# arangesh/Ground-Plane-Polling

Hardware: AMD Instinct MI355X
Metric: images/sec end-to-end (resnet50, 1k planes, 1242x375) (higher is better)
Workload: dtype f16x3

## Files before the change

### ground-plane-polling_amd/csrc/conv_igemm.hip

```cpp

#include <hip/hip_runtime.h>
#include <stdint.h>
#include <stdlib.h>

#include "conv_igemm_types.h"
#include "gpp.h"

namespace {

inline bool is_x3(int dtype) { return dtype == GPP_BF16X3 || dtype == GPP_F16X3; }
inline bool f32_storage(int dtype) { return dtype == GPP_F32 || is_x3(dtype); }
inline int elem_size(int dtype) { return f32_storage(dtype) ? 4 : 2; }

int validate(const gpp_conv_desc& d)
{
    if (!d.in || !d.weight || !d.out) return GPP_ERR_BAD_ARG;
    if (d.dtype != GPP_BF16 && d.dtype != GPP_F16 && d.dtype != GPP_F32 && !is_x3(d.dtype)) return GPP_ERR_UNSUPPORTED;
    const int esz = elem_size(d.dtype), ck = 128 / esz, va = 16 / esz;
    if (d.batch <= 0 || d.C_in <= 0 || d.C_out <= 0 || d.KH <= 0 || d.KW <= 0) return GPP_ERR_BAD_ARG;
    constexpr int kMaxDim = 1 << 20;
    if (d.batch > kMaxDim || d.C_in > kMaxDim || d.C_out > kMaxDim || d.in_pitch > kMaxDim || d.out_pitch > kMaxDim || d.res_pitch > kMaxDim ||
        d.weight_rows > kMaxDim || d.weight_rows < 0 || d.in_pitch < 0 || d.out_pitch < 0 || d.res_pitch < 0 || d.partial_bytes < 0)
        return GPP_ERR_UNSUPPORTED;
    if (d.KH > 8 || d.KW > 8) return GPP_ERR_UNSUPPORTED;
// ... 138 lines not shown
{
    return block_entry(conv1x1_a, conv3x3_b, conv1x1_c, tile, stream);
}

extern "C" int gpp_bottleneck_tail(const gpp_conv_desc* conv3x3, const gpp_conv_desc* conv1x1, int tile_rows, void* stream)
{
    return tail_entry(conv3x3, conv1x1, tile_rows, stream);
}

extern "C" int gpp_x3_range_events(uint64_t* host_count, int reset)
{
    unsigned long long v = 0;
    const int rc = gpp_x3_range_events_f16x3(&v, reset);
    if (rc == GPP_OK && host_count) *host_count = (uint64_t)v;
    return rc;
}

extern "C" int gpp_x3_range_snapshot(uint64_t* device_count, void* stream)
{
    return gpp_x3_range_snapshot_of(nullptr, device_count, stream);
}

extern "C" int gpp_x3_range_snapshot_of(const uint64_t* counter, uint64_t* device_count, void* stream)
{
    if (!device_count) return GPP_ERR_BAD_ARG;
    if (((uintptr_t)counter | (uintptr_t)device_count) & 7) return GPP_ERR_ALIGN;
    return gpp_x3_range_snapshot_f16x3((const unsigned long long*)counter, (unsigned long long*)device_count, (hipStream_t)stream);
}

extern "C" int gpp_conv2d_flops(const gpp_conv_desc* host_desc, double* flops)
{
    if (!host_desc || !flops) return GPP_ERR_BAD_ARG;
    if (host_desc->n_groups < 1 || host_desc->n_groups > GPP_MAX_GROUPS) return GPP_ERR_BAD_ARG;
    double f = 0.0;
    for (int g = 0; g < host_desc->n_groups; ++g)
        f += 2.0 * host_desc->batch * (double)host_desc->groups[g].H_out * host_desc->groups[g].W_out *
             host_desc->KH * host_desc->KW * (double)host_desc->C_in * host_desc->C_out;
    *flops = f;
    return GPP_OK;
}

extern "C" int gpp_conv2d_split_rule(const gpp_conv_desc* host_desc, int* split_k)
{
    if (!host_desc || !split_k) return GPP_ERR_BAD_ARG;
    gpp_conv_desc d = *host_desc;
    int rc = validate(d);
    if (rc != GPP_OK) return rc;
    *split_k = d.split_k > 0 ? d.split_k : split_rule(d);
    return GPP_OK;
}

extern "C" int gpp_conv2d_workspace_bytes(const gpp_conv_desc* host_desc, size_t* bytes)
{
    if (!host_desc || !bytes) return GPP_ERR_BAD_ARG;
    gpp_conv_desc d = *host_desc;
    char probe[16] __attribute__((aligned(16)));
    if (!d.partial) { d.partial = probe; d.partial_bytes = 0; }
    int rc = validate(d);
    if (rc != GPP_OK) return rc;
    const int split = d.split_k > 0 ? d.split_k : split_rule(d);
    *bytes = 0;
    if (split <= 1) return GPP_OK;
    int64_t rows = 0;
    for (int g = 0; g < d.n_groups; ++g) rows += (int64_t)d.batch * d.groups[g].H_out * d.groups[g].W_out + 256;
    const int64_t npad = (d.C_out + 255) / 256 * 256;
    *bytes = (size_t)(split * rows * npad * 4);
    return GPP_OK;
}

extern "C" int gpp_conv2d_igemm(const gpp_conv_desc* host_desc, void* stream)
{
    if (!host_desc) return GPP_ERR_BAD_ARG;
    gpp_conv_desc d = *host_desc;
    for (int g = 0; g < GPP_MAX_GROUPS; ++g) d.groups[g].row_begin = 0;
    int rc = validate(d);
    if (rc != GPP_OK) return rc;
    return dispatch_any(d, (hipStream_t)stream);
}

static const int kTiles[] = {0, 64064, 96064, 128064, 160064, 192064, 64128, 96128, 128128, 160128, 192128, 224128,
                             1128128, 1192128, 1128256, 1160256, 1192256, 1224256, 256256, 1256256,
                             128160, 192160, 1192160, 1128160, 2256256, 1192096, 3256224, 3192160, 4128064, 4064064, 4128128, 4064128,
                             5064064, 5096064, 5064128, 5096128, 5128128,
                             128256, 192256};
static bool tile_is_candidate(const gpp_conv_desc* desc, int tile)
{
    const int ck = 128 / elem_size(desc->dtype);
    const int nk = desc->KH * desc->KW * (desc->C_in / ck);
    int64_t rows = 0;
    for (int g = 0; g < desc->n_groups; ++g) rows += (int64_t)desc->batch * desc->groups[g].H_out * desc->groups[g].W_out;
    const int bn = tile % 1000 ? tile % 1000 : 128;
    if (tile >= 5000000) {
        static const bool no_deep = [] { const char* e = getenv("GPP_NO_DEEP_TILES"); return e && e[0] == '1'; }();
        const bool x3_in = is_x3(desc->dtype) && (desc->x3_split & GPP_X3_IN);
        const int bm = (tile / 1000) % 1000;
        int64_t tiles_m = 0;
        for (int g = 0; g < desc->n_groups; ++g) tiles_m += ((int64_t)desc->batch * desc->groups[g].H_out * desc->groups[g].W_out + bm - 1) / bm;
        const int64_t wgs = tiles_m * ((desc->C_out + bn - 1) / bn) * (desc->split_k > 1 ? desc->split_k : 1);
        if (bn == 64 && desc->C_out > 256) return false;
        return !no_deep && x3_in && nk >= 12 && wgs <= 320;
    }
    if (tile >= 4000000) {
        static const bool no_ws = [] { const char* e = getenv("GPP_NO_WS_TILES"); return e && e[0] == '1'; }();
        const bool x3_in = is_x3(desc->dtype) && (desc->x3_split & GPP_X3_IN);
        const int bm = (tile / 1000) % 1000;
        const gpp_conv_group& G = desc->groups[0];
        return !no_ws && x3_in && desc->KH == 1 && desc->KW == 1 && desc->stride == 1 && desc->pad_top == 0 && desc->pad_left == 0 && desc->n_groups == 1 &&
               desc->split_k <= 1 && desc->C_out % bn == 0 && 32 % (desc->C_out / bn) == 0 && G.H_in == G.H_out && G.W_in == G.W_out &&
               (!desc->residual || ((desc->x3_split & GPP_X3_RES) && G.H_res == G.H_out && G.W_res == G.W_out)) &&
               (desc->C_in / 32) * bn * 128 + 4 * bm * 128 <= 160 * 1024 && rows >= 256 * 16;
    }
    static const bool no_mix = [] { const char* e = getenv("GPP_NO_MIX_TILES"); return e && e[0] == '1'; }();
    if (tile >= 3000000 && no_mix) return false;
    if (tile >= 3000000) {
        const bool x3_in = is_x3(desc->dtype) && (desc->x3_split & GPP_X3_IN);
        return x3_in && desc->C_out % 256 == 0 && nk >= 4 && desc->split_k <= 1 && rows * (desc->C_out / 256) >= 256 * 256;
    }
    if (tile && bn == 64 && desc->C_out > 256 && !(desc->KH == 1 && desc->KW == 1 && desc->C_in <= 256)) return false;
    if (bn == 256 && (desc->C_out < 192 || rows < 256 * 16)) return false;
    const bool x3_pipe = is_x3(desc->dtype) && (desc->x3_split & GPP_X3_IN);
    if (tile > 1000000 && tile < 3000000 && (nk < 4 || (f32_storage(desc->dtype) && !x3_pipe))) return false;
    if ((tile == 1256256 || tile == 1160256 || tile == 1224256) && !x3_pipe) return false;
    if (x3_pipe && tile == 1192160) return false;
    if (bn == 256 && desc->dtype == GPP_F32) return false;
    if ((tile == 128256 || tile == 192256) && !is_x3(desc->dtype)) return false;
    if (bn == 160 && (desc->C_out + 159) / 160 * 160 >= (desc->C_out + 127) / 128 * 128) return false;
    if (bn == 96 && (desc->C_out + 95) / 96 * 96 >= (desc->C_out + 127) / 128 * 128) return false;
    if (tile == 2256256 && (desc->C_out < 384 || desc->C_out % 256 != 128 || rows < 256 * 16)) return false;
    return true;
}

extern "C" int gpp_conv2d_tile_candidates(const gpp_conv_desc* desc, int* tiles, int capacity, int* count)
{
    if (!desc || !count || capacity < 0 || (capacity > 0 && !tiles)) return GPP_ERR_BAD_ARG;
    {
        gpp_conv_desc d = *desc;
        for (int g = 0; g < GPP_MAX_GROUPS; ++g) d.groups[g].row_begin = 0;
        const int rc = validate(d);
        if (rc != GPP_OK) return rc;
    }
    int n = 0;
    for (int tile : kTiles) {
        if (!tile_is_candidate(desc, tile)) continue;
        if (n < capacity) tiles[n] = tile;
        ++n;
    }
    *count = n;
    return GPP_OK;
}

extern "C" int gpp_conv2d_autotune(gpp_conv_desc* desc, int iters, void* stream, float* best_us)
{
    if (!desc || iters < 1) return GPP_ERR_BAD_ARG;
    {
        gpp_conv_desc d = *desc;
        for (int g = 0; g < GPP_MAX_GROUPS; ++g) d.groups[g].row_begin = 0;
        const int rc = validate(d);
        if (rc != GPP_OK) return rc;
    }
    hipStream_t st = (hipStream_t)stream;
    hipEvent_t e0, e1;
    hipError_t e = hipEventCreate(&e0);
    if (e != hipSuccess) return (int)e;
    e = hipEventCreate(&e1);
    if (e != hipSuccess) { (void)hipEventDestroy(e0); return (int)e; }
    const int tile_in = desc->tile_hint;
    float best = 1e30f;
    int best_tile = tile_in, rc = GPP_OK;
    auto time_one = [&](int tile, float* us, int reps = 2) -> int {
        desc->tile_hint = tile;
        int r = gpp_conv2d_igemm(desc, stream);
        if (r != GPP_OK) return r;
        float t_best = 1e30f;
        for (int rep = 0; rep < reps; ++rep) {
// ... 41 lines not shown
```

### ground-plane-polling_amd/csrc/conv_igemm_impl.h

```cpp
#ifndef GPP_CONV_IGEMM_IMPL_H_
#define GPP_CONV_IGEMM_IMPL_H_

#include <hip/hip_runtime.h>
#include <stdint.h>

#include <atomic>

#include "gpp.h"

namespace {

typedef __attribute__((ext_vector_type(8))) __bf16 bf16x8;
typedef __attribute__((ext_vector_type(8))) _Float16 f16x8;
typedef __attribute__((ext_vector_type(4))) float f32x4;

struct f32x8 {
    f32x4 lo, hi;
    __device__ __forceinline__ float operator[](int e) const { return e < 4 ? lo[e] : hi[e - 4]; }
};

template <int DT> struct Elem;
template <> struct Elem<GPP_BF16> {
    using scalar = __bf16;
    using vec8 = bf16x8;
// ... 1769 lines not shown
    };
    rows_of(0, obase, rbase, valid);
    fetch_res(rbase);

    f32x4 acc[MF][NF];
    for (int c = 0; c < my_tiles; ++c) {
#pragma unroll
        for (int i = 0; i < MF; ++i)
#pragma unroll
            for (int j = 0; j < NF; ++j) acc[i][j] = (f32x4){0.f, 0.f, 0.f, 0.f};
        int slot = (c * nk) & (R - 1);
        for (int ks = 0; ks < nk; ++ks) {
            if (ks == 0) asm volatile("s_waitcnt vmcnt(0)" ::: "memory");
            else asm volatile("s_waitcnt vmcnt(%0)" ::"n"((D - 1) * A_IT) : "memory");
            asm volatile("s_waitcnt lgkmcnt(0)" ::: "memory");
            __builtin_amdgcn_s_barrier();
            asm volatile("" ::: "memory");
            issue();
            const unsigned char* sa = ring + slot * SLAB;
            const unsigned char* sw = wbase + ks * BN * kRowBytes;
            xh8 ah[MF], al[MF], bh[NF], bl[NF];
#pragma unroll
            for (int i = 0; i < MF; ++i) {
                ah[i] = *(const xh8*)(sa + a_rd[0] + i * 16 * kRowBytes);
                al[i] = *(const xh8*)(sa + a_rd[1] + i * 16 * kRowBytes);
            }
#pragma unroll
            for (int j = 0; j < NF; ++j) {
                bh[j] = *(const xh8*)(sw + b_rd[0] + j * 16 * kRowBytes);
                bl[j] = *(const xh8*)(sw + b_rd[1] + j * 16 * kRowBytes);
            }
#pragma unroll
            for (int i = 0; i < MF; ++i)
#pragma unroll
                for (int j = 0; j < NF; ++j) {
                    const int js = GPP_SERP2(i, j, NF);
                    acc[i][js] = X3Half<DT>::mfma(bl[js], ah[i], acc[i][js]);
                    acc[i][js] = X3Half<DT>::mfma(bh[js], ah[i], acc[i][js]);
                }
#pragma unroll
            for (int i = 0; i < MF; ++i)
#pragma unroll
                for (int j = 0; j < NF; ++j) { const int js = GPP_SERP2(i, j, NF); acc[i][js] = X3Half<DT>::mfma(bh[js], al[i], acc[i][js]); }
            slot = (slot + 1) & (R - 1);
        }
        float v[MF][NG][8];
#pragma unroll
        for (int i = 0; i < MF; ++i)
#pragma unroll
            for (int jj = 0; jj < NG; ++jj) {
#pragma unroll
                for (int e = 0; e < 4; ++e) {
                    if constexpr (OSCALE) {
                        v[i][jj][e] = __builtin_fmaf(acc[i][2 * jj][e], scale_v[jj][e], bias_v[jj][e]);
                        v[i][jj][4 + e] = __builtin_fmaf(acc[i][2 * jj + 1][e], scale_v[jj][4 + e], bias_v[jj][4 + e]);
                    } else {
                        v[i][jj][e] = acc[i][2 * jj][e] + bias_v[jj][e];
                        v[i][jj][4 + e] = acc[i][2 * jj + 1][e] + bias_v[jj][4 + e];
                    }
                }
                if constexpr (HASRES) {
                    float r[8];
                    x3_unpack<DT>(rpre[i][jj].lo, rpre[i][jj].hi, r);
#pragma unroll
                    for (int e = 0; e < 8; ++e) v[i][jj][e] += r[e];
                }
            }
        int64_t ob_next[MF], rb_next[MF];
        bool ok_next[MF];
        if (c + 1 < my_tiles) {
            rows_of(c + 1, ob_next, rb_next, ok_next);
            fetch_res(rb_next);
        }
#pragma unroll
        for (int i = 0; i < MF; ++i)
            if (valid[i]) {
#pragma unroll
                for (int jj = 0; jj < NG; ++jj) finish8_pre<DT>(d, v[i][jj], n + 32 * jj, obase[i], false, f32x8());
            }
        if (c + 1 < my_tiles) {
#pragma unroll
            for (int i = 0; i < MF; ++i) { obase[i] = ob_next[i]; rbase[i] = rb_next[i]; valid[i] = ok_next[i]; }
        }
    }
}

struct DeviceOnce {
    std::atomic<uint64_t> mask{0};
    template <typename K>
    int configure(K kernel, int lds)
    {
        int dev = 0;
        hipError_t e = hipGetDevice(&dev);
        if (e != hipSuccess) return (int)e;
        const uint64_t bit = 1ull << (dev & 63);
        if (mask.load(std::memory_order_acquire) & bit) return GPP_OK;
        e = hipFuncSetAttribute((const void*)kernel, hipFuncAttributeMaxDynamicSharedMemorySize, lds);
        if (e != hipSuccess) return (int)e;
        mask.fetch_or(bit, std::memory_order_release);
        return GPP_OK;
    }
};

template <int DT, int BM, int BN, int WM, int WN, int STAGES, bool PIPE, bool XIN = false>
int launch(gpp_conv_desc& d, hipStream_t st)
{
    if constexpr (kX3<DT> && !XIN) {
        if (d.x3_split & GPP_X3_IN) return launch<DT, BM, BN, WM, WN, STAGES, PIPE, true>(d, st);
    }
    constexpr int BMS = stage_rows(BM, WM * WN);
    constexpr int lds = STAGES * (BMS + BN) * kRowBytes;
    constexpr int CK = kRowBytes / Elem<DT>::ESZ;
    static DeviceOnce once;
    auto kernel = conv_igemm_kernel<DT, BM, BN, WM, WN, STAGES, PIPE, XIN>;
    int rc = once.configure(kernel, lds);
    if (rc != GPP_OK) return rc;
    const int tiles = prepare<BM, BN>(d);
    if (tiles < 0) return tiles;
    const int n_tiles = (d.C_out + BN - 1) / BN;
    const int nk = d.KH * d.KW * (d.C_in / CK);
    int nsplit = 1;
    if (d.split_k > 1) {
        nsplit = d.split_k;
        if (nk / nsplit < 1) return GPP_ERR_BAD_ARG;
        const int64_t slab = (int64_t)tiles * BM * n_tiles * BN * 4;
        if (!d.partial || slab * nsplit > (int64_t)d.partial_bytes) return GPP_ERR_WORKSPACE;
    }
    const int steps = (nk + nsplit - 1) / nsplit;
    const int lds_used = PIPE ? lds : (steps < STAGES ? steps : STAGES) * (BMS + BN) * kRowBytes;
    kernel<<<dim3((unsigned)(tiles * n_tiles), (unsigned)nsplit), dim3(64 * WM * WN), lds_used, st>>>(d);
    if (nsplit > 1) {
        const int64_t total = (int64_t)d.partial_rows * ((d.C_out + 7) / 8);
        splitk_reduce_kernel<DT><<<dim3((unsigned)((total + 255) / 256)), dim3(256), 0, st>>>(d, BM, n_tiles * BN, nsplit);
    }
    hipError_t e = hipGetLastError();
    return e == hipSuccess ? GPP_OK : (int)e;
}

template <int DT>
int launch_dual(const gpp_conv_desc& d, hipStream_t st)
{
    constexpr bool X3 = kX3<DT>;
    constexpr int ESZ = Elem<DT>::ESZ, CK = kRowBytes / ESZ;
    if (X3 && !(d.x3_split & GPP_X3_IN)) return GPP_ERR_UNSUPPORTED;
    if (d.C_out < 384 || d.C_out % 256 != 128 || d.KH * d.KW * (d.C_in / CK) < 2 || d.split_k > 1) return GPP_ERR_UNSUPPORTED;
    constexpr int lds = 2 * (512 + 128) * kRowBytes;
    static DeviceOnce once;
    auto kernel = conv_igemm_dual_kernel<DT, X3>;
    int rc = once.configure(kernel, lds);
    if (rc != GPP_OK) return rc;
    const int head = d.C_out - 128;
    gpp_conv_desc d0 = d, d1 = d;
    d0.C_out = head;
    d1.C_out = 128;
    d1.weight = (const char*)d.weight + (int64_t)head * d.KH * d.KW * d.C_in * ESZ;
    d1.weight_rows = d.weight_rows - head;
    if (d.bias) d1.bias = d.bias + head;
    if (d.out_scale) d1.out_scale = d.out_scale + head;
    for (int g = 0; g < d.n_groups; ++g) {
        d1.groups[g].out_off += head;
        d1.groups[g].res_off += head;
    }
    const int t0 = prepare<256, 256>(d0), t1 = prepare<512, 128>(d1);
    if (t0 < 0) return t0;
    if (t1 < 0) return t1;
    const int n0 = t0 * (head / 256), n1 = t1;
// ... 4 lines not shown
}

template <int DT, int BMA, int BMB>
int launch_mix(const gpp_conv_desc& d, hipStream_t st)
{
    constexpr int BN = 256, CUS = 256;
    constexpr int ESZ = Elem<DT>::ESZ, CK = kRowBytes / ESZ;
    static_assert(kX3<DT>, "mixed grids exist for the x3 types");
    if (!(d.x3_split & GPP_X3_IN)) return GPP_ERR_UNSUPPORTED;
    if (d.C_out % BN != 0 || d.KH * d.KW * (d.C_in / CK) < 2 || d.split_k > 1) return GPP_ERR_UNSUPPORTED;
    const int n_tiles = d.C_out / BN;
    const int64_t rows0 = (int64_t)d.batch * d.groups[0].H_out * d.groups[0].W_out;
    auto tiles_b = [&](int64_t begin, int bm) {
        int64_t t = (rows0 - begin + bm - 1) / bm;
        for (int g = 1; g < d.n_groups; ++g) t += ((int64_t)d.batch * d.groups[g].H_out * d.groups[g].W_out + bm - 1) / bm;
        return t * n_tiles;
    };
    int64_t best_cost = (tiles_b(0, BMA) + CUS - 1) / CUS * BMA;
    int best_ra = 0;
    for (int ra = 1; ra <= 64; ++ra) {
        if ((ra * CUS) % n_tiles != 0) continue;
        const int64_t ma = (int64_t)ra * CUS / n_tiles;
        if (ma * BMA > rows0) break;
        const int64_t cost = (int64_t)ra * BMA + (tiles_b(ma * BMA, BMB) + CUS - 1) / CUS * BMB;
        if (cost < best_cost) { best_cost = cost; best_ra = ra; }
    }
    if (best_ra == 0) return GPP_ERR_UNSUPPORTED;
    constexpr int lds = 2 * (stage_rows(BMA > BMB ? BMA : BMB, 8) + BN) * kRowBytes;
    static DeviceOnce once;
    auto kernel = conv_igemm_mix_kernel<DT, BMA, BMB, BN, true>;
    int rc = once.configure(kernel, lds);
    if (rc != GPP_OK) return rc;
    const int ma = best_ra * CUS / n_tiles;
    gpp_conv_desc da = d, db = d;
    da.n_groups = 1;
    const int ta = prepare<BMA, BN>(da);
    if (ta < 0) return ta;
    db.groups[0].row_begin = ma * BMA;
    const int tb = prepare<BMB, BN>(db);
    if (tb < 0) return tb;
    da.in_bytes = db.in_bytes;
    const int na = ma * n_tiles, nb = tb * n_tiles;
    const int splita = (na + 7) / 8 * 8;
    kernel<<<dim3((unsigned)(splita + nb)), dim3(512), lds, st>>>(da, db, na, splita, nb);
    hipError_t e = hipGetLastError();
    return e == hipSuccess ? GPP_OK : (int)e;
}

template <int DT, int BM, int BN>
int launch_ws(gpp_conv_desc& d, hipStream_t st)
{
    constexpr int R = 4;
    static_assert(kX3<DT>, "weight-stationary 1 x 1: x3 types");
    const gpp_conv_group& G = d.groups[0];
    if (!(d.x3_split & GPP_X3_IN) || d.KH != 1 || d.KW != 1 || d.stride != 1 || d.pad_top != 0 || d.pad_left != 0 || d.n_groups != 1 || d.split_k > 1)
        return GPP_ERR_UNSUPPORTED;
    if (d.C_out % BN != 0 || 32 % (d.C_out / BN) != 0 || d.C_in % 32 != 0) return GPP_ERR_UNSUPPORTED;
    if (G.H_in != G.H_out || G.W_in != G.W_out) return GPP_ERR_UNSUPPORTED;
    if (d.residual && (!(d.x3_split & GPP_X3_RES) || G.H_res != G.H_out || G.W_res != G.W_out)) return GPP_ERR_UNSUPPORTED;
    const int nk = d.C_in / 32;
    const int lds = nk * BN * kRowBytes + R * BM * kRowBytes;
    if (lds > 160 * 1024) return GPP_ERR_UNSUPPORTED;
    const int tiles = prepare<BM, BN>(d);
    if (tiles < 0) return tiles;
    const int n_mtiles = (int)(((int64_t)d.batch * G.H_out * G.W_out + BM - 1) / BM);
    int rc;
    if (d.residual) {
        static DeviceOnce once;
        auto kernel = conv1x1_ws_kernel<DT, BM, BN, true>;
        rc = once.configure(kernel, 160 * 1024);
        if (rc != GPP_OK) return rc;
        kernel<<<dim3(256), dim3(512), lds, st>>>(d, n_mtiles);
    } else {
        static DeviceOnce once;
        auto kernel = conv1x1_ws_kernel<DT, BM, BN, false>;
        rc = once.configure(kernel, 160 * 1024);
        if (rc != GPP_OK) return rc;
        kernel<<<dim3(256), dim3(512), lds, st>>>(d, n_mtiles);
    }
    hipError_t e = hipGetLastError();
    return e == hipSuccess ? GPP_OK : (int)e;
}

template <int DT>
int dispatch(gpp_conv_desc& d, hipStream_t st)
{
    switch (d.tile_hint) {
        case 64:
        case 128064: return launch<DT, 128, 64, 2, 2, 2, false>(d, st);
        case 64064: return launch<DT, 64, 64, 2, 2, 2, false>(d, st);
        case 96064: return launch<DT, 96, 64, 2, 2, 2, false>(d, st);
        case 160064: return launch<DT, 160, 64, 2, 2, 2, false>(d, st);
        case 192064: return launch<DT, 192, 64, 2, 2, 2, false>(d, st);
        case 64128: return launch<DT, 64, 128, 2, 2, 2, false>(d, st);
        case 96128: return launch<DT, 96, 128, 2, 2, 2, false>(d, st);
        case 128:
        case 128128:
#ifdef GPP_STAMPS
            if constexpr (!kF32Storage<DT>) if (d.reserved & 4) return launch<DT, 128, 128, 2, 2, 2, true>(d, st);
#endif
            return launch<DT, 128, 128, 2, 2, 2, false>(d, st);
        case 160128: return launch<DT, 160, 128, 2, 2, 2, false>(d, st);
        case 192128: return launch<DT, 192, 128, 2, 2, 2, false>(d, st);
        case 224128: return launch<DT, 224, 128, 2, 2, 2, false>(d, st);
        case 128160: return launch<DT, 128, 160, 4, 1, 2, false>(d, st);
        case 192160:
            if constexpr (kX3<DT>) {
                if (!(d.x3_split & GPP_X3_IN)) return GPP_ERR_UNSUPPORTED;
                return launch<DT, 192, 160, 4, 1, 2, false, true>(d, st);
            } else {
                return launch<DT, 192, 160, 4, 1, 2, false>(d, st);
            }
        case 0: break;
        default:
            if constexpr (!kF32Storage<DT>) {
                switch (d.tile_hint) {
                    case 256: return launch<DT, 256, 128, 4, 2, 3, false>(d, st);
                    case 1128128: return launch<DT, 128, 128, 2, 2, 2, true>(d, st);
                    case 1192128: return launch<DT, 192, 128, 2, 2, 2, true>(d, st);
                    case 1128256: return launch<DT, 128, 256, 2, 4, 2, true>(d, st);
                    case 1192256: return launch<DT, 192, 256, 2, 4, 2, true>(d, st);
                    case 1192160: return launch<DT, 192, 160, 4, 1, 2, true>(d, st);
                    case 1128160: return launch<DT, 128, 160, 4, 1, 2, true>(d, st);
                    case 1192096: return launch<DT, 192, 96, 4, 1, 2, true>(d, st);
                    case 2256256: return launch_dual<DT>(d, st);
                    case 512:
                    case 256256:
#ifdef GPP_STAMPS
                        if (d.reserved & 8) return launch<DT, 256, 256, 2, 4, 2, false>(d, st);
#endif
                        return launch<DT, 256, 256, 2, 4, 2, true>(d, st);
                    default: return GPP_ERR_BAD_ARG;
                }
            } else {
                if constexpr (kX3<DT>) {
                    if (d.x3_split & GPP_X3_IN) {
                        switch (d.tile_hint) {
                            case 1256256: return launch<DT, 256, 256, 2, 4, 2, true, true>(d, st);
                            case 1224256: return launch<DT, 224, 256, 2, 4, 2, true, true>(d, st);
                            case 1192256: return launch<DT, 192, 256, 2, 4, 2, true, true>(d, st);
                            case 1160256: return launch<DT, 160, 256, 2, 4, 2, true, true>(d, st);
                            case 1128256: return launch<DT, 128, 256, 2, 4, 2, true, true>(d, st);
                            case 1192128: return launch<DT, 192, 128, 2, 2, 2, true, true>(d, st);
                            case 1128128: return launch<DT, 128, 128, 2, 2, 2, true, true>(d, st);
                            case 1128160: return launch<DT, 128, 160, 4, 1, 2, true, true>(d, st);
                            case 1192096: return launch<DT, 192, 96, 4, 1, 2, true, true>(d, st);
                            case 2256256: return launch_dual<DT>(d, st);
                            case 3256224: return launch_mix<DT, 256, 224>(d, st);
                            case 3192160: return launch_mix<DT, 192, 160>(d, st);
                            case 4128064: return launch_ws<DT, 128, 64>(d, st);
                            case 4064064: return launch_ws<DT, 64, 64>(d, st);
                            case 4128128: return launch_ws<DT, 128, 128>(d, st);
                            case 4064128: return launch_ws<DT, 64, 128>(d, st);
                            case 5064064: return launch<DT, 64, 64, 2, 2, 4, false, true>(d, st);
                            case 5096064: return launch<DT, 96, 64, 2, 2, 4, false, true>(d, st);
                            case 5064128: return launch<DT, 64, 128, 2, 2, 4, false, true>(d, st);
                            case 5096128: return launch<DT, 96, 128, 2, 2, 4, false, true>(d, st);
                            case 5128128: return launch<DT, 128, 128, 2, 2, 4, false, true>(d, st);
                            default: break;
                        }
                    }
                    if (d.tile_hint == 256256) return launch<DT, 256, 256, 2, 4, 2, false>(d, st);
                    if (d.tile_hint == 192256) return launch<DT, 192, 256, 2, 4, 2, false>(d, st);
                    if (d.tile_hint == 128256) return launch<DT, 128, 256, 2, 4, 2, false>(d, st);
                }
                switch (d.tile_hint) {
                    case 256: case 1128128: case 1192128: case 1128256: case 1192256: case 1192160: case 1128160: case 2256256: case 512: case 256256: case 1256256:
                    case 192256: case 128256: case 1192096: case 3256224: case 3192160: case 1224256: case 1160256: case 4128064: case 4064064: case 4128128: case 4064128:
                    case 5064064: case 5096064: case 5064128: case 5096128: case 5128128:
                        return GPP_ERR_UNSUPPORTED;
                    default: return GPP_ERR_BAD_ARG;
                }
            }
    }
    if (d.C_out <= 64 || (d.C_out % 128 != 0 && d.C_out % 128 <= 64)) return launch<DT, 128, 64, 2, 2, 2, false>(d, st);
    if constexpr (!kF32Storage<DT>) {
        int64_t rows = 0;
        for (int g = 0; g < d.n_groups; ++g) rows += (int64_t)d.batch * d.groups[g].H_out * d.groups[g].W_out;
        const int nk = d.KH * d.KW * (d.C_in / 64);
        const int n256 = (d.C_out + 255) / 256;
        const int64_t big_blocks = ((rows + 255) / 256) * n256;
        const bool n_fits = d.C_out >= 256 && n256 * 256 * 7 <= d.C_out * 8;
        if (n_fits && big_blocks >= 512 && nk >= 8 && d.split_k <= 1) return launch<DT, 256, 256, 2, 4, 2, true>(d, st);
    }
    return launch<DT, 128, 128, 2, 2, 2, false>(d, st);
}

template <int DT, int BM, int CMID>
int launch_tail(gpp_conv_desc& d1, gpp_conv_desc& d2, hipStream_t st)
{
    constexpr int lds = 2 * (BM + CMID) * kRowBytes;
    static DeviceOnce once;
    auto kernel = bottleneck_tail_kernel<DT, BM, CMID>;
    int rc = once.configure(kernel, lds);
    if (rc != GPP_OK) return rc;
    const gpp_conv_group& G = d1.groups[0];
    const int64_t in_elems = G.in_off + (int64_t)(d1.batch - 1) * G.in_bstride + ((int64_t)G.H_in * G.W_in - 1) * d1.in_pitch + d1.C_in;
    const int64_t w1_bytes = (int64_t)d1.weight_rows * 9 * CMID * 2, w2_bytes = (int64_t)d2.weight_rows * CMID * 2;
    if (G.in_off < 0 || G.in_bstride < 0 || in_elems * 2 >= (1LL << 31) || w1_bytes >= (1LL << 31) || w2_bytes >= (1LL << 31))
        return GPP_ERR_UNSUPPORTED;
    d1.in_bytes = (int32_t)(in_elems * 2);
    d1.weight_bytes = (int32_t)w1_bytes;
    d2.weight_bytes = (int32_t)w2_bytes;
    const int64_t rows = (int64_t)d1.batch * G.H_out * G.W_out;
    kernel<<<dim3((unsigned)((rows + BM - 1) / BM)), dim3(256), lds, st>>>(d1, d2);
    hipError_t e = hipGetLastError();
    return e == hipSuccess ? GPP_OK : (int)e;
}

template <int DT, int BM, int CMID>
int launch_tail_x3(gpp_conv_desc& d1, gpp_conv_desc& d2, hipStream_t st)
{
    constexpr int KC = CMID / 32;
    constexpr int ring = 2 * (BM + CMID) * kRowBytes, phase2 = KC * BM * kRowBytes + KC * 128 * kRowBytes;
    constexpr int lds = ring > phase2 ? ring : phase2;
    static DeviceOnce once;
    auto kernel = bottleneck_tail_x3_kernel<DT, BM, CMID>;
    int rc = once.configure(kernel, lds);
    if (rc != GPP_OK) return rc;
    const gpp_conv_group& G = d1.groups[0];
    const int64_t in_elems = G.in_off + (int64_t)(d1.batch - 1) * G.in_bstride + ((int64_t)G.H_in * G.W_in - 1) * d1.in_pitch + d1.C_in;
    const int64_t w1_bytes = (int64_t)d1.weight_rows * 9 * CMID * 4, w2_bytes = (int64_t)d2.weight_rows * CMID * 4;
    if (G.in_off < 0 || G.in_bstride < 0 || in_elems * 4 >= (1LL << 31) || w1_bytes >= (1LL << 31) || w2_bytes >= (1LL << 31))
        return GPP_ERR_UNSUPPORTED;
    d1.in_bytes = (int32_t)(in_elems * 4);
    d1.weight_bytes = (int32_t)w1_bytes;
    d2.weight_bytes = (int32_t)w2_bytes;
    const int64_t rows = (int64_t)d1.batch * G.H_out * G.W_out;
    kernel<<<dim3((unsigned)((rows + BM - 1) / BM)), dim3(256), lds, st>>>(d1, d2);
    hipError_t e = hipGetLastError();
    return e == hipSuccess ? GPP_OK : (int)e;
}

template <int DT>
int dispatch_tail_x3(gpp_conv_desc& d1, gpp_conv_desc& d2, int tile_rows, hipStream_t st)
{
    if (d1.C_in != 64) return GPP_ERR_UNSUPPORTED;
    switch (tile_rows) {
        case 64: return launch_tail_x3<DT, 64, 64>(d1, d2, st);
        case 96: return launch_tail_x3<DT, 96, 64>(d1, d2, st);
        case 0:
        case 128: return launch_tail_x3<DT, 128, 64>(d1, d2, st);
        case 160: return launch_tail_x3<DT, 160, 64>(d1, d2, st);
        default: return GPP_ERR_BAD_ARG;
    }
}

template <int DT>
int dispatch_tail(gpp_conv_desc& d1, gpp_conv_desc& d2, int tile_rows, hipStream_t st)
{
    const bool c64 = d1.C_in == 64;
    switch (tile_rows) {
// ... 12 lines not shown
```

### ground-plane-polling_amd/keras_retinanet_3D/models/retinanet.py

```python

import ctypes
import json
import os

import numpy as np

from ..backend import hip
from ..layers import conv as C
from ..layers.filter_detections import MAX_DETECTIONS, NMS_THRESHOLD, SCORE_THRESHOLD
from ..utils import anchors as anchor_utils
from ..utils.gpp_utils import POLL_THRESHOLD
from . import weights as W


class StemDesc(ctypes.Structure):
    _fields_ = [('inp', ctypes.c_void_p), ('weight', ctypes.c_void_p), ('bias', ctypes.c_void_p), ('out', ctypes.c_void_p),
                ('dtype', ctypes.c_int32), ('B', ctypes.c_int32), ('H', ctypes.c_int32), ('W', ctypes.c_int32), ('range_counter', ctypes.c_void_p)]


class PoolDesc(ctypes.Structure):
    _fields_ = [('inp', ctypes.c_void_p), ('out', ctypes.c_void_p), ('dtype', ctypes.c_int32), ('B', ctypes.c_int32),
                ('H', ctypes.c_int32), ('W', ctypes.c_int32), ('C', ctypes.c_int32), ('reserved', ctypes.c_int32)]


# ... 457 lines not shown
            plan.regression, reg_o = pyramid(144, torch.float32)
            self._conv(plan, 'pyramid_regression_ops', reg_t, reg_o, 3, pad=(1, 1), out_f32=True, join=bool(cls_lane))

        detect_at = {}
        if overlap:
            cls_tower()
            detect_at['candidates'] = len(plan.ops)
            reg_tower()
            detect_at['select'] = len(plan.ops)
            dim_tower()
        else:
            dim_tower()
            cls_tower()
            reg_tower()

        D = MAX_DETECTIONS
        f32, i32 = torch.float32, torch.int32
        plan.boxes = torch.empty((B, D, 12), dtype=f32, device=dev)
        plan.dimensions = torch.empty((B, D, 3), dtype=f32, device=dev)
        plan.scores = torch.empty((B, D), dtype=f32, device=dev)
        plan.labels = torch.empty((B, D), dtype=i32, device=dev)
        plan.orientations = torch.empty((B, D), dtype=i32, device=dev)
        plan.anchor_index = torch.empty((B, D), dtype=i32, device=dev)
        plan.counts = torch.zeros((B,), dtype=i32, device=dev)
        need = hip.c_size_t(0)
        if self.osf and B > 16:
            raise ValueError('orientation_specific_filter=True handles at most 16 images per batch')
        size_fn = hip.lib().gpp_detect_osf_workspace_bytes if self.osf else hip.lib().gpp_detect_workspace_bytes
        hip.check(size_fn(B, plan.n_anchors, need), 'gpp_detect_workspace_bytes')
        plan.detect_ws = torch.empty((int(need.value),), dtype=torch.uint8, device=dev)
        anchors = self._anchor_table((H, Wd))
        dd = DetectDesc(plan.cls_logits.data_ptr(), plan.regression.data_ptr(), plan.regression_dim.data_ptr(),
                        anchors.data_ptr(), plan.boxes.data_ptr(), plan.dimensions.data_ptr(), plan.scores.data_ptr(),
                        plan.labels.data_ptr(), plan.orientations.data_ptr(), plan.anchor_index.data_ptr(),
                        plan.counts.data_ptr(), plan.detect_ws.data_ptr(), plan.detect_ws.numel(), plan.n_anchors,
                        B, anchor_utils.NUM_BASE_ANCHORS, 1, D, SCORE_THRESHOLD, NMS_THRESHOLD if self.nms else 2.0)
        sp = Plan.span_of
        det_out = [sp(t) for t in (plan.boxes, plan.dimensions, plan.scores, plan.labels, plan.orientations, plan.anchor_index)]
        heads_in = [sp(plan.cls_logits), sp(plan.regression), sp(plan.regression_dim)]
        plan.touch(dd, [sp(plan.cls_logits)], [sp(plan.detect_ws), sp(plan.counts)], kind=OP_DETECT_CANDIDATES)
        plan.touch(dd, [sp(plan.detect_ws), sp(plan.regression)], [sp(plan.detect_ws)], kind=OP_DETECT_SELECT)
        plan.touch(dd, heads_in + [sp(plan.detect_ws)], det_out, kind=OP_DETECT_EMIT)
        for whole in (OP_DETECT, OP_DETECT_OSF):
            plan.touch(dd, heads_in, det_out + [sp(plan.detect_ws), sp(plan.counts)], kind=whole)
        if overlap:
            at = detect_at['select']
            plan.ops.insert(at, (OP_DETECT_SELECT, 0, dd, 'filtered_detections/select', 0.0))
            plan.lanes.insert(at, (1 << 8) | OP_SYNC)
            at = detect_at['candidates']
            plan.ops.insert(at, (OP_DETECT_CANDIDATES, 0, dd, 'filtered_detections/candidates', 0.0))
            plan.lanes.insert(at, (cls_lane or 1) << 8)
            plan.add(OP_DETECT_EMIT, dd, 'filtered_detections', join=True)
        else:
            plan.add(OP_DETECT_OSF if self.osf else OP_DETECT, dd, 'filtered_detections', join=True)

        plan.keypoints = torch.empty((B, D, 4, 3), dtype=f32, device=dev)
        plan.keyplanes = torch.empty((B, D, 1, 4), dtype=f32, device=dev)
        plan.residuals = torch.empty((B, D), dtype=f32, device=dev)
        plan.best_index = torch.empty((B, D), dtype=i32, device=dev)
        hip.check(hip.lib().gpp_poll_workspace_bytes(B, n_planes, int(planes_batched), need), 'gpp_poll_workspace_bytes')
        plan.poll_ws = torch.empty((max(int(need.value), 16),), dtype=torch.uint8, device=dev)
        pd = PollDesc(plan.boxes.data_ptr(), plan.dimensions.data_ptr(), plan.orientations.data_ptr(), plan.P_inv.data_ptr(),
                      plan.planes.data_ptr(), plan.keypoints.data_ptr(), plan.keyplanes.data_ptr(), plan.residuals.data_ptr(),
                      plan.best_index.data_ptr(), plan.poll_ws.data_ptr(), plan.poll_ws.numel(), B, D, n_planes,
                      int(planes_batched), POLL_THRESHOLD, 0)
        plan.add(OP_POLL, pd, 'fit_road_planes', tag=2, flops=162.0 * B * D * n_planes)
        plan.touch(pd, [Plan.span_of(t) for t in (plan.boxes, plan.dimensions, plan.orientations, plan.P_inv, plan.planes)],
                   [Plan.span_of(t) for t in (plan.keypoints, plan.keyplanes, plan.residuals, plan.best_index, plan.poll_ws)])
        plan.workspaces = {lane: torch.empty((max(need_, 16),), dtype=torch.uint8, device=dev) for lane, need_ in plan.ws_need.items()}
        for d, lane in plan.conv_descs:
            d.partial = plan.workspaces[lane].data_ptr()
            d.partial_bytes = plan.workspaces[lane].numel()
        plan.finalize()
        plan.tagged = [name for _, tag, _, name, _ in plan.ops if tag]
        if os.environ.get('GPP_AUTOTUNE', '1') != '0':
            self._autotune(plan)
        return plan

    def _tune_cache_path(self):
        return os.environ.get('GPP_TUNE_CACHE')

    def _tune_config(self):
        ver = hip.lib().gpp_version().decode().split('src:')[-1]
        return 'v2;{};x3split={};fuse={};plan={}{}'.format(ver, os.environ.get('GPP_X3_SPLIT', '2'), os.environ.get('GPP_FUSE_TAIL', '64,128') + '/' + os.environ.get('GPP_FUSE_BLOCK', '64,128'), self.plan_mode,
                                                           C.latency_split_config() if self.plan_mode == 'latency' else '')

    def _load_tune_cache(self):
        path = self._tune_cache_path()
        if path and os.path.exists(path):
            with open(path) as f:
                for key, val in json.load(f).items():
                    parts = key.split('|')
                    if len(parts) != 7:
                        continue
                    cfg, bb, dt, name, b, h, w = parts
                    if cfg == self._tune_config() and bb == self.backbone_name and dt == self.dtype:
                        self._tuned[(name, int(b), int(h), int(w))] = (int(val[0]), float(val[-1]))

    def _save_tune_cache(self):
        path = self._tune_cache_path()
        if not path or int(os.environ.get('RANK', '0')) != 0:
            return
        data = {}
        if os.path.exists(path):
            try:
                with open(path) as f:
                    data = json.load(f)
            except ValueError:
                data = {}
        for (name, b, h, w), val in self._tuned.items():
            data['|'.join([self._tune_config(), self.backbone_name, self.dtype, name, str(b), str(h), str(w)])] = list(val)
        tmp = '{}.tmp.{}'.format(path, os.getpid())
        with open(tmp, 'w') as f:
            json.dump(data, f, indent=0, sort_keys=True)
        os.replace(tmp, path)

    def _autotune(self, plan):
        torch = self.torch
        B, H, Wd = plan.shape[:3]
        plan.images.uniform_(-120.0, 130.0)
        best = ctypes.c_float(0.0)
        fresh = False
        plan.tuning = {}
        rnd = None
        if os.environ.get('GPP_TUNE_RANDOM'):
            import random
            rnd = random.Random(int(os.environ['GPP_TUNE_RANDOM']) * 1000003 + int(os.environ.get('RANK', '0')))
        for index, (kind, _, desc, name, flops) in enumerate(plan.ops):
            if kind in DETECT_OPS or kind == OP_POLL:
                continue
            self.run_op(plan, index)
            if rnd is not None and kind in (OP_TAIL, OP_CONV):
                if kind == OP_CONV:
                    tiles, count = (ctypes.c_int * 32)(), ctypes.c_int(0)
                    hip.check(hip.lib().gpp_conv2d_tile_candidates(ctypes.byref(desc), tiles, 32, ctypes.byref(count)), 'gpp_conv2d_tile_candidates')
                    ok = []
                    for tile in tiles[:count.value]:
                        desc.tile_hint = tile
                        if hip.lib().gpp_plan_run(ctypes.byref(plan.array, index * ctypes.sizeof(PlanOp)), 1, hip.stream_ptr(), None, 0) == 0:
                            ok.append(tile)
                    desc.tile_hint = rnd.choice(ok)
                    plan.tuning[name] = (int(desc.tile_hint), 0.0)
                else:
                    desc.tile_rows = rnd.choice((64, 96, 128, 160) if self.dtype in C.X3_TYPES else (96, 128, 160))
                    plan.tuning[name] = (int(desc.tile_rows), 0.0)
                self.run_op(plan, index)
                continue
            if kind == OP_TAIL:
                key = (name, plan.op_batch.get(id(desc), B), H, Wd)
                if key not in self._tuned:
                    times = {}
                    for rows in ((64, 96, 128, 160) if (self.dtype in C.X3_TYPES and os.environ.get('GPP_TAIL64', '1') != '0') else (96, 128, 160)):
                        desc.tile_rows = rows
                        e0, e1 = torch.cuda.Event(enable_timing=True), torch.cuda.Event(enable_timing=True)
                        self.run_op(plan, index)
                        e0.record()
                        for _ in range(16):
                            self.run_op(plan, index)
                        e1.record()
                        e1.synchronize()
                        times[rows] = e0.elapsed_time(e1) * 1000.0 / 16
                    rows = min(times, key=times.get)
                    self._tuned[key] = (rows, round(times[rows], 2))
                    fresh = True
                desc.tile_rows = self._tuned[key][0]
                plan.tuning[name] = self._tuned[key]
                plan.tuning_parts.setdefault(name, []).append(self._tuned[key])
                continue
# ... 239 lines not shown
```

Before: 823.9.

## Add persistent x3 implicit-GEMM conv kernel with cross-tile prefetch as autotune candidates

Adds a persistent conv kernel for x3 dtypes. Each workgroup walks several (m, n, split) tiles assigned per XCD, and it issues the next tile's global-to-LDS loads while finishing the current tile's epilogue. The kernel comes in five tile shapes and is exposed as new autotune candidates for convs with at most 32768 output rows. The aim is to remove per-tile launch and tail latency and to hide pipeline fill on small layers. The cost is more code, a larger autotune search, and an env var to switch it off, which is also folded into the tune-cache key.

```diff
diff --git a/ground-plane-polling_amd/csrc/conv_igemm.hip b/ground-plane-polling_amd/csrc/conv_igemm.hip
--- a/ground-plane-polling_amd/csrc/conv_igemm.hip
+++ b/ground-plane-polling_amd/csrc/conv_igemm.hip
@@ -244,7 +244,8 @@
                              1128128, 1192128, 1128256, 1160256, 1192256, 1224256, 256256, 1256256,
                              128160, 192160, 1192160, 1128160, 2256256, 1192096, 3256224, 3192160, 4128064, 4064064, 4128128, 4064128,
                              5064064, 5096064, 5064128, 5096128, 5128128,
-                             128256, 192256};
+                             128256, 192256,
+                             6064064, 6096064, 6064128, 6096128, 6160064};
 static bool tile_is_candidate(const gpp_conv_desc* desc, int tile)
 {
     const int ck = 128 / elem_size(desc->dtype);
@@ -252,6 +253,12 @@
     int64_t rows = 0;
     for (int g = 0; g < desc->n_groups; ++g) rows += (int64_t)desc->batch * desc->groups[g].H_out * desc->groups[g].W_out;
     const int bn = tile % 1000 ? tile % 1000 : 128;
+    if (tile >= 6000000) {
+        static const bool no_persist = [] { const char* e = getenv("GPP_NO_PERSIST_TILES"); return e && e[0] == '1'; }();
+        const bool x3_in = is_x3(desc->dtype) && (desc->x3_split & GPP_X3_IN);
+        if (bn == 64 && desc->C_out > 256) return false;
+        return !no_persist && x3_in && desc->C_out % 8 == 0 && rows <= 32768;
+    }
     if (tile >= 5000000) {
         static const bool no_deep = [] { const char* e = getenv("GPP_NO_DEEP_TILES"); return e && e[0] == '1'; }();
         const bool x3_in = is_x3(desc->dtype) && (desc->x3_split & GPP_X3_IN);
diff --git a/ground-plane-polling_amd/csrc/conv_igemm_impl.h b/ground-plane-polling_amd/csrc/conv_igemm_impl.h
--- a/ground-plane-polling_amd/csrc/conv_igemm_impl.h
+++ b/ground-plane-polling_amd/csrc/conv_igemm_impl.h
@@ -1875,6 +1875,326 @@
 #pragma unroll
             for (int i = 0; i < MF; ++i) { obase[i] = ob_next[i]; rbase[i] = rb_next[i]; valid[i] = ok_next[i]; }
         }
+    }
+}
+
+template <int DT, int BM, int BN, int WM, int WN, int STAGES>
+__global__ __launch_bounds__(64 * WM * WN, 2) void conv_igemm_persist_kernel(const gpp_conv_desc d, const int n_items, const int nsplit)
+{
+    static_assert(kX3<DT>, "x3 types on pre-split input maps");
+    using E = Elem<DT>;
+    using vec8 = typename E::vec8;
+    using xh8 = typename X3Half<DT>::vec;
+    constexpr int ESZ = E::ESZ, CK = kRowBytes / ESZ;
+    constexpr int NW = WM * WN;
+    constexpr int MF = BM / WM / 16, NF = BN / WN / 16;
+    constexpr int BMS = stage_rows(BM, NW);
+    constexpr int A_BYTES = BMS * kRowBytes, B_BYTES = BN * kRowBytes, STAGE = A_BYTES + B_BYTES;
+    constexpr int A_IT = BMS / 8 / NW, B_IT = BN / 8 / NW;
+    constexpr int PER_STAGE = A_IT + B_IT;
+    constexpr int PF = STAGES - 1;
+    constexpr int COLS = BN / WN;
+    constexpr bool OSCALE = (DT == GPP_F16X3);
+    static_assert(MF >= 1 && NF % 2 == 0 && A_IT >= 1 && B_IT >= 1 && BMS % (8 * NW) == 0 && BN % (8 * NW) == 0 && BM % (16 * WM) == 0, "tile / wave shape");
+    static_assert(STAGES >= 2 && STAGES * STAGE <= 80 * 1024, "two workgroups per CU");
+
+    extern __shared__ __attribute__((aligned(16))) unsigned char smem[];
+    const int tid = threadIdx.x, lane = tid & 63;
+    const int wave = __builtin_amdgcn_readfirstlane(tid >> 6);
+    const int wm = wave / WN, wn = wave % WN;
+    const int frow = lane & 15, fq = lane >> 4;
+
+    const int xcd = blockIdx.x & 7, local = blockIdx.x >> 3, q = gridDim.x >> 3;
+    const int Q = n_items >> 3, r8 = n_items & 7;
+    const int lo = xcd < r8 ? xcd * (Q + 1) : r8 * (Q + 1) + (xcd - r8) * Q;
+    const int hi = lo + Q + (xcd < r8 ? 1 : 0);
+    int f = lo + local;
+    if (f >= hi) return;
+
+    const int n_tiles = (d.C_out + BN - 1) / BN;
+    const int tiles_nm = n_items / nsplit;
+    const int Ktot = d.KH * d.KW * d.C_in;
+    const int cpt = d.C_in / CK;
+    const int nk_total = d.KH * d.KW * cpt;
+    const int taps = d.KH * d.KW;
+    const int pitch2 = d.in_pitch * ESZ;
+    const int srow = lane >> 3, gchunk = (lane & 7) ^ srow;
+    const __amdgpu_buffer_rsrc_t in_rsrc = __builtin_amdgcn_make_buffer_rsrc((void*)d.in, 0, d.in_bytes, 0x00020000);
+    const __amdgpu_buffer_rsrc_t w_rsrc = __builtin_amdgcn_make_buffer_rsrc((void*)d.weight, 0, d.weight_bytes, 0x00020000);
+
+    struct Geo {
+        int tile_start, row_begin, H_in, W_in, H_out, W_out, H_res, W_res;
+        int64_t in_off, in_bs, out_off, out_bs, res_off, res_bs;
+    };
+    auto geo_of = [&](int mt) {
+        Geo g = {};
+#pragma unroll
+        for (int k = 0; k < GPP_MAX_GROUPS; ++k) {
+            if (k < d.n_groups && mt >= d.groups[k].tile_start) {
+                g.tile_start = d.groups[k].tile_start;
+                g.row_begin = d.groups[k].row_begin;
+                g.H_in = d.groups[k].H_in; g.W_in = d.groups[k].W_in;
+                g.H_out = d.groups[k].H_out; g.W_out = d.groups[k].W_out;
+                g.H_res = d.groups[k].H_res; g.W_res = d.groups[k].W_res;
+                g.in_off = d.groups[k].in_off; g.in_bs = d.groups[k].in_bstride;
+                g.out_off = d.groups[k].out_off; g.out_bs = d.groups[k].out_bstride;
+                g.res_off = d.groups[k].res_off; g.res_bs = d.groups[k].res_bstride;
+            }
+        }
+        return g;
+    };
+    struct Item { int split, mt, nt, ks0, nk; };
+    auto item_of = [&](int fi) {
+        Item it;
+        it.split = fi / tiles_nm;
+        const int bid = fi - it.split * tiles_nm;
+        it.nt = bid % n_tiles;
+        it.mt = bid / n_tiles;
+        it.ks0 = 0;
+        it.nk = nk_total;
+        if (nsplit > 1) {
+            it.ks0 = (int)((unsigned)(nk_total * it.split) / (unsigned)nsplit);
+            it.nk = (int)((unsigned)(nk_total * (it.split + 1)) / (unsigned)nsplit) - it.ks0;
+        }
+        return it;
+    };
+
+    int a_base[A_IT], a_mask[A_IT], a_voff[A_IT], w_voff[B_IT];
+    int i_W_in = 0, i_ks0 = 0, i_nk = 0, issued = 0, cc = 0, kh = 0, kw = 0, ibuf = 0;
+    auto set_tap = [&](int kh_, int kw_) {
+        const int delta = (kh_ * i_W_in + kw_) * pitch2;
+        const int need = (1 << kh_) | (1 << (8 + kw_));
+#pragma unroll
+        for (int i = 0; i < A_IT; ++i) a_voff[i] = ((a_mask[i] & need) == need) ? a_base[i] + delta : kOutOfRange;
+    };
+    auto setup_issue = [&](int fi) {
+        const Item it = item_of(fi);
+        const Geo g = geo_of(it.mt);
+        const int HoWo = g.H_out * g.W_out, Mg = d.batch * HoWo;
+        const int m0 = g.row_begin + (it.mt - g.tile_start) * BM, n0 = it.nt * BN;
+        PixWalk pw;
+        pw.init(m0 + wave * A_IT * 8 + srow, HoWo, g.W_out);
+#pragma unroll
+        for (int i = 0; i < A_IT; ++i) {
+            const int m = m0 + (wave * A_IT + i) * 8 + srow;
+            a_mask[i] = 0;
+            a_base[i] = 0;
+            if (m < Mg) {
+                const int iy0 = pw.oy * d.stride - d.pad_top, ix0 = pw.ox * d.stride - d.pad_left;
+                const int rlo = max(0, -iy0), rhi = min(d.KH, max(0, g.H_in - iy0));
+                const int clo = max(0, -ix0), chi = min(d.KW, max(0, g.W_in - ix0));
+                const int rmask = rhi > rlo ? ((1 << rhi) - 1) & ~((1 << rlo) - 1) : 0;
+                const int cmask = chi > clo ? ((1 << chi) - 1) & ~((1 << clo) - 1) : 0;
+                a_mask[i] = rmask | (cmask << 8);
+                a_base[i] = (int)((g.in_off + (int64_t)pw.b * g.in_bs) * ESZ) + gchunk * 16 + (iy0 * g.W_in + ix0) * pitch2;
+            }
+            if (i + 1 < A_IT) pw.advance(8, g.H_out, g.W_out);
+        }
+#pragma unroll
+        for (int i = 0; i < B_IT; ++i) w_voff[i] = (n0 + (wave * B_IT + i) * 8 + srow) * Ktot * ESZ + gchunk * 16;
+        i_W_in = g.W_in;
+        i_ks0 = it.ks0;
+        i_nk = it.nk;
+        issued = 0;
+        cc = it.ks0 / taps;
+        kw = (it.ks0 % taps) % d.KW;
+        kh = (it.ks0 % taps) / d.KW;
+        set_tap(kh, kw);
+    };
+    auto issue_next = [&]() {
+        unsigned char* sa = smem + ibuf * STAGE + wave * A_IT * 8 * kRowBytes;
+        unsigned char* sb = smem + ibuf * STAGE + A_BYTES + wave * B_IT * 8 * kRowBytes;
+#pragma unroll
+        for (int i = 0; i < A_IT; ++i) glds16(in_rsrc, a_voff[i], cc * kRowBytes, sa + i * 8 * kRowBytes);
+#pragma unroll
+        for (int i = 0; i < B_IT; ++i) glds16(w_rsrc, w_voff[i], (i_ks0 + issued) * kRowBytes, sb + i * 8 * kRowBytes);
+        if (++kw == d.KW) {
+            kw = 0;
+            if (++kh == d.KH) { kh = 0; ++cc; }
+        }
+        set_tap(kh, kw);
+        ++issued;
+        if (++ibuf == STAGES) ibuf = 0;
+    };
+    auto issue_first = [&]() {
+#pragma unroll
+        for (int p = 0; p < PF; ++p)
+            if (issued < i_nk) issue_next();
+    };
+
+    int a_rd[2], b_rd[2];
+#pragma unroll
+    for (int kk = 0; kk < 2; ++kk) {
+        const int sw = ((kk * 4 + fq) ^ (frow & 7)) << 4;
+        a_rd[kk] = (wm * (BM / WM) + frow) * kRowBytes + sw;
+        b_rd[kk] = A_BYTES + (wn * (BN / WN) + frow) * kRowBytes + sw;
+    }
+
+    f32x4 acc[MF][NF];
+    vec8 rpre[MF][NF / 2];
+    RowAddr ra[MF];
+    float bias_v[NF / 2][8];
+    float scale_v[OSCALE ? NF / 2 : 1][8];
+    const bool has_res = d.residual != nullptr && nsplit == 1;
+    int cbuf = 0;
+
+    setup_issue(f);
+    issue_first();
+    for (;;) {
+        const Item it = item_of(f);
+        const Geo g = geo_of(it.mt);
+        const int HoWo = g.H_out * g.W_out, Mg = d.batch * HoWo;
+        const int m0 = g.row_begin + (it.mt - g.tile_start) * BM, n0 = it.nt * BN;
+        const int nk = it.nk;
+        if (nsplit == 1) {
+#pragma unroll
+            for (int jj = 0; jj < NF / 2; ++jj) {
+                const int n = n0 + wn * COLS + jj * 32 + fq * 8;
+#pragma unroll
+                for (int e = 0; e < 8; ++e) bias_v[jj][e] = (d.bias && n + e < d.C_out) ? d.bias[n + e] : 0.0f;
+                if constexpr (OSCALE) {
+#pragma unroll
+                    for (int e = 0; e < 8; ++e) scale_v[jj][e] = (d.out_scale && n + e < d.C_out) ? d.out_scale[n + e] : 1.0f;
+                }
+            }
+            PixWalk pw;
+            pw.init(m0 + wm * (BM / WM) + frow, HoWo, g.W_out);
+            const PixWalk first = {0, 0, 0};
+#pragma unroll
+            for (int i = 0; i < MF; ++i) {
+                const int m = m0 + wm * (BM / WM) + i * 16 + frow;
+                ra[i] = row_addr_at(d, m < Mg ? pw : first, g.W_out, g.H_out, g.H_res, g.W_res, g.out_off, g.out_bs, g.res_off, g.res_bs);
+                if (i + 1 < MF) pw.advance(16, g.H_out, g.W_out);
+                if (has_res) {
+#pragma unroll
+                    for (int jj = 0; jj < NF / 2; ++jj) {
+                        const int n = n0 + wn * COLS + jj * 32 + fq * 8;
+                        const int nc = n < d.C_out ? n : 0;
+                        if (d.x3_split & GPP_X3_RES) {
+                            const char* p = x3_addr(d.residual, ra[i].rbase, nc);
+                            rpre[i][jj].lo = *(const f32x4*)p;
+                            rpre[i][jj].hi = *(const f32x4*)(p + 64);
+                        } else {
+                            rpre[i][jj] = *(const vec8*)((const float*)d.residual + ra[i].rbase + nc);
+                        }
+                    }
+                }
+            }
+        }
+#pragma unroll
+        for (int i = 0; i < MF; ++i)
+#pragma unroll
+            for (int j = 0; j < NF; ++j) acc[i][j] = (f32x4){0.f, 0.f, 0.f, 0.f};
+
+        for (int ks = 0; ks < nk; ++ks) {
+            if (issued - ks - 1 >= PF - 1 && PF > 1)
+                asm volatile("s_waitcnt vmcnt(%0)" ::"n"((PF - 1) * PER_STAGE) : "memory");
+            else
+                asm volatile("s_waitcnt vmcnt(0)" ::: "memory");
+            asm volatile("s_waitcnt lgkmcnt(0)" ::: "memory");
+            __builtin_amdgcn_s_barrier();
+            asm volatile("" ::: "memory");
+            if (issued < nk) issue_next();
+            const unsigned char* sbase = smem + cbuf * STAGE;
+            xh8 ah[MF], al[MF], bh[NF], bl[NF];
+#pragma unroll
+            for (int i = 0; i < MF; ++i) {
+                ah[i] = *(const xh8*)(sbase + a_rd[0] + i * 16 * kRowBytes);
+                al[i] = *(const xh8*)(sbase + a_rd[1] + i * 16 * kRowBytes);
+            }
+#pragma unroll
+            for (int j = 0; j < NF; ++j) {
+                bh[j] = *(const xh8*)(sbase + b_rd[0] + j * 16 * kRowBytes);
+                bl[j] = *(const xh8*)(sbase + b_rd[1] + j * 16 * kRowBytes);
+            }
+#pragma unroll
+            for (int i = 0; i < MF; ++i)
+#pragma unroll
+                for (int j = 0; j < NF; ++j) {
+                    const int js = GPP_SERP2(i, j, NF);
+                    acc[i][js] = X3Half<DT>::mfma(bl[js], ah[i], acc[i][js]);
+                    acc[i][js] = X3Half<DT>::mfma(bh[js], ah[i], acc[i][js]);
+                }
+#pragma unroll
+            for (int i = 0; i < MF; ++i)
+#pragma unroll
+                for (int j = 0; j < NF; ++j) { const int js = GPP_SERP2(i, j, NF); acc[i][js] = X3Half<DT>::mfma(bh[js], al[i], acc[i][js]); }
+            if (++cbuf == STAGES) cbuf = 0;
+        }
+
+        const int fn = f + q;
+        const bool more = fn < hi;
+        if (more) setup_issue(fn);
+
+        if (nsplit > 1) {
+            if (more) issue_first();
+            const int64_t rows_pad = (int64_t)d.partial_rows, npad = (int64_t)n_tiles * BN;
+            float* part = (float*)d.partial + ((int64_t)it.split * rows_pad + (int64_t)it.mt * BM) * npad + it.nt * BN;
+#pragma unroll
+            for (int i = 0; i < MF; ++i) {
+                const int lr = wm * (BM / WM) + i * 16 + frow;
+#pragma unroll
+                for (int jj = 0; jj < NF / 2; ++jj) {
+                    float* dst = part + (int64_t)lr * npad + wn * COLS + jj * 32 + fq * 8;
+                    *(f32x4*)dst = acc[i][2 * jj];
+                    *(f32x4*)(dst + 4) = acc[i][2 * jj + 1];
+                }
+            }
+        } else {
+#pragma unroll
+            for (int i = 0; i < MF; ++i) {
+#pragma unroll
+                for (int jj = 0; jj < NF / 2; ++jj) {
+                    float v[8];
+#pragma unroll
+                    for (int e = 0; e < 4; ++e) {
+                        if constexpr (OSCALE) {
+                            v[e] = acc[i][2 * jj][e] * scale_v[jj][e] + bias_v[jj][e];
+                            v[4 + e] = acc[i][2 * jj + 1][e] * scale_v[jj][4 + e] + bias_v[jj][4 + e];
+                        } else {
+                            v[e] = acc[i][2 * jj][e] + bias_v[jj][e];
+                            v[4 + e] = acc[i][2 * jj + 1][e] + bias_v[jj][4 + e];
+                        }
+                    }
+                    if (has_res) {
+                        float rv[8];
+                        if (d.x3_split & GPP_X3_RES) {
+                            x3_unpack<DT>(rpre[i][jj].lo, rpre[i][jj].hi, rv);
+                        } else {
+#pragma unroll
+                            for (int e = 0; e < 8; ++e) rv[e] = rpre[i][jj][e];
+                        }
+#pragma unroll
+                        for (int e = 0; e < 8; ++e) v[e] += rv[e];
+                    }
+#pragma unroll
+                    for (int e = 0; e < 4; ++e) {
+                        acc[i][2 * jj][e] = v[e];
+                        acc[i][2 * jj + 1][e] = v[4 + e];
+                    }
+                }
+            }
+            if (more) issue_first();
+#pragma unroll
+            for (int i = 0; i < MF; ++i) {
+                const int m = m0 + wm * (BM / WM) + i * 16 + frow;
+                if (m >= Mg) break;
+#pragma unroll
+                for (int jj = 0; jj < NF / 2; ++jj) {
+                    const int n = n0 + wn * COLS + jj * 32 + fq * 8;
+                    if (n >= d.C_out) continue;
+                    float v[8];
+#pragma unroll
+                    for (int e = 0; e < 4; ++e) {
+                        v[e] = acc[i][2 * jj][e];
+                        v[4 + e] = acc[i][2 * jj + 1][e];
+                    }
+                    finish8<DT>(d, v, n, ra[i].obase, nullptr);
+                }
+            }
+        }
+        if (!more) break;
+        f = fn;
     }
 }
 
@@ -2045,6 +2365,40 @@
     return e == hipSuccess ? GPP_OK : (int)e;
 }
 
+template <int DT, int BM, int BN, int STAGES>
+int launch_persist(gpp_conv_desc& d, hipStream_t st)
+{
+    static_assert(kX3<DT>, "persistent x3 tiles");
+    constexpr int WM = 2, WN = 2, CUS = 256;
+    constexpr int lds = STAGES * (stage_rows(BM, WM * WN) + BN) * kRowBytes;
+    if (!(d.x3_split & GPP_X3_IN) || d.C_out % 8 != 0) return GPP_ERR_UNSUPPORTED;
+    static DeviceOnce once;
+    auto kernel = conv_igemm_persist_kernel<DT, BM, BN, WM, WN, STAGES>;
+    int rc = once.configure(kernel, lds);
+    if (rc != GPP_OK) return rc;
+    const int tiles = prepare<BM, BN>(d);
+    if (tiles < 0) return tiles;
+    const int n_tiles = (d.C_out + BN - 1) / BN;
+    const int nk = d.KH * d.KW * (d.C_in / 32);
+    int nsplit = 1;
+    if (d.split_k > 1) {
+        nsplit = d.split_k;
+        if (nk / nsplit < 1) return GPP_ERR_BAD_ARG;
+        const int64_t slab = (int64_t)tiles * BM * n_tiles * BN * 4;
+        if (!d.partial || slab * nsplit > (int64_t)d.partial_bytes) return GPP_ERR_WORKSPACE;
+    }
+    const int64_t items = (int64_t)tiles * n_tiles * nsplit;
+    if (items >= (1LL << 30)) return GPP_ERR_UNSUPPORTED;
+    const int64_t grid = items < 2 * CUS ? (items + 7) / 8 * 8 : 2 * CUS;
+    kernel<<<dim3((unsigned)grid), dim3(64 * WM * WN), lds, st>>>(d, (int)items, nsplit);
+    if (nsplit > 1) {
+        const int64_t total = (int64_t)d.partial_rows * ((d.C_out + 7) / 8);
+        splitk_reduce_kernel<DT><<<dim3((unsigned)((total + 255) / 256)), dim3(256), 0, st>>>(d, BM, n_tiles * BN, nsplit);
+    }
+    hipError_t e = hipGetLastError();
+    return e == hipSuccess ? GPP_OK : (int)e;
+}
+
 template <int DT>
 int dispatch(gpp_conv_desc& d, hipStream_t st)
 {
@@ -2093,6 +2447,8 @@
                         if (d.reserved & 8) return launch<DT, 256, 256, 2, 4, 2, false>(d, st);
 #endif
                         return launch<DT, 256, 256, 2, 4, 2, true>(d, st);
+                    case 6064064: case 6096064: case 6064128: case 6096128: case 6160064:
+                        return GPP_ERR_UNSUPPORTED;
                     default: return GPP_ERR_BAD_ARG;
                 }
             } else {
@@ -2120,6 +2476,11 @@
                             case 5064128: return launch<DT, 64, 128, 2, 2, 4, false, true>(d, st);
                             case 5096128: return launch<DT, 96, 128, 2, 2, 4, false, true>(d, st);
                             case 5128128: return launch<DT, 128, 128, 2, 2, 4, false, true>(d, st);
+                            case 6064064: return launch_persist<DT, 64, 64, 4>(d, st);
+                            case 6096064: return launch_persist<DT, 96, 64, 4>(d, st);
+                            case 6064128: return launch_persist<DT, 64, 128, 3>(d, st);
+                            case 6096128: return launch_persist<DT, 96, 128, 2>(d, st);
+                            case 6160064: return launch_persist<DT, 160, 64, 2>(d, st);
                             default: break;
                         }
                     }
@@ -2131,6 +2492,7 @@
                     case 256: case 1128128: case 1192128: case 1128256: case 1192256: case 1192160: case 1128160: case 2256256: case 512: case 256256: case 1256256:
                     case 192256: case 128256: case 1192096: case 3256224: case 3192160: case 1224256: case 1160256: case 4128064: case 4064064: case 4128128: case 4064128:
                     case 5064064: case 5096064: case 5064128: case 5096128: case 5128128:
+                    case 6064064: case 6096064: case 6064128: case 6096128: case 6160064:
                         return GPP_ERR_UNSUPPORTED;
                     default: return GPP_ERR_BAD_ARG;
                 }
diff --git a/ground-plane-polling_amd/keras_retinanet_3D/models/retinanet.py b/ground-plane-polling_amd/keras_retinanet_3D/models/retinanet.py
--- a/ground-plane-polling_amd/keras_retinanet_3D/models/retinanet.py
+++ b/ground-plane-polling_amd/keras_retinanet_3D/models/retinanet.py
@@ -563,8 +563,9 @@
 
     def _tune_config(self):
         ver = hip.lib().gpp_version().decode().split('src:')[-1]
-        return 'v2;{};x3split={};fuse={};plan={}{}'.format(ver, os.environ.get('GPP_X3_SPLIT', '2'), os.environ.get('GPP_FUSE_TAIL', '64,128') + '/' + os.environ.get('GPP_FUSE_BLOCK', '64,128'), self.plan_mode,
-                                                           C.latency_split_config() if self.plan_mode == 'latency' else '')
+        return 'v2;{};x3split={};fuse={};plan={}{}{}'.format(ver, os.environ.get('GPP_X3_SPLIT', '2'), os.environ.get('GPP_FUSE_TAIL', '64,128') + '/' + os.environ.get('GPP_FUSE_BLOCK', '64,128'), self.plan_mode,
+                                                             C.latency_split_config() if self.plan_mode == 'latency' else '',
+                                                             ';nopersist' if os.environ.get('GPP_NO_PERSIST_TILES', '0') == '1' else '')
 
     def _load_tune_cache(self):
         path = self._tune_cache_path()
```

After: 823.2, median of 3. About the same (-0.1%).
